# navallo/collision_avoidance

Measured on AMD Instinct MI355X. Metric: agent-steps/sec (whole node), 4096 arenas x 64 agents per GPU, higher is better.
Workload: dtype f32

## Files before the change

### collision_avoidance_amd/csrc/ca_obs.h

```cpp
#pragma once
#include "ca_common.h"

namespace ca {

struct ObsArgs {
    const float *pos_x, *pos_y, *vel_x, *vel_y, *orient_x, *orient_y;
    const unsigned short* counts;
    const void* nb_idx;
    const unsigned short* obst_idx;
    const ObstDev* obst;
    const int* tab_off;
    float* obs;
    int A, N, K, S, bpa;
    int nstage_max;
    int paircap;
    int a0;
    int xcd;
    int dense;
    unsigned long long* dbg;
    float radius;
    float rays[32];
    float oct[32];
    const float* ap_oct;
    const int* agent_counts;
};

#ifdef CA_STAMPS
#define CA_OSTAMP(k)                                                                       \
    do {                                                                                   \
        __builtin_amdgcn_sched_barrier(0);                                                 \
        const unsigned long long _t = CA_STAMP_CLOCK();                                    \
        __builtin_amdgcn_s_waitcnt(0xC07F);                                                \
        if ((threadIdx.x & 63) == 0 && p.dbg)                                              \
            p.dbg[((size_t)blockIdx.x * (blockDim.x >> 6) + (threadIdx.x >> 6)) * 16 + (k)] = _t; \
        __builtin_amdgcn_sched_barrier(0);                                                 \
    } while (0)
#else
#define CA_OSTAMP(k) do { } while (0)
#endif

__host__ __device__ inline size_t obs_lds_bytes(int nstage_max, int obs_bs, int paircap, int obw = 16) {
    const size_t apb = obs_bs / 16;
    return (size_t)nstage_max * 16 + 2 * apb * 16 * 8 + apb * 16 + apb * 16 * 4 + apb * (size_t)obw * 4 + 64 * 4 + 2 * apb * 4 + apb * (size_t)paircap * 2;
}
__host__ __device__ inline size_t obs_lds_bytes_ap(int nstage_max, int obs_bs, int paircap) {
    return ((obs_lds_bytes(nstage_max, obs_bs, paircap) + 15) & ~(size_t)15) + (size_t)(obs_bs / 16) * 16 * 64;
}
#ifndef CA_OBS_BS_MAX
#define CA_OBS_BS_MAX 256
#endif
__host__ __device__ inline int obs_block_threads(int N) {
    const int want = N > 32 ? 1024 : (N > 16 ? 512 : 256);
    return want < CA_OBS_BS_MAX ? want : CA_OBS_BS_MAX;
}

struct SegGeom {
    float s02x, s02y;
    float s32x, s32y;
    float t_numer;
    float r1x, r1y, r2x, r2y;
};

__device__ __forceinline__ float ray_dial(float x, float y) {
    const float yy = -y;
    const float ax = fabsf(x), ay = fabsf(yy);
    const float mx = fmaxf(ax, ay), mn = fminf(ax, ay);
    const float a = mn * __builtin_amdgcn_rcpf(mx);
    const float s = a * a;
    float r = a * (0.99997726f + s * (-0.33262347f + s * (0.19354346f + s * (-0.11643287f +
              s * (0.05265332f + s * -0.01172120f)))));
    r = (ay > ax) ? 1.57079632679f - r : r;
    r = (x < 0.0f) ? 3.14159265359f - r : r;
    r = (yy < 0.0f) ? -r : r;
    const float u = r * 2.54647908947f;
    return (u < 0.0f) ? u + 16.0f : u;
}

template <int OBS_BS, bool NW16, bool DENSE = false, class... WIDE_TAG>
__global__ __launch_bounds__(OBS_BS) void obs_kernel(const ObsArgs p) {
    constexpr bool WIDE = has_tag<WideObstLists, WIDE_TAG...>;
    constexpr bool AC = has_tag<ArenaCounts, WIDE_TAG...>;
    constexpr bool AP = has_tag<AgentParams, WIDE_TAG...> || AC;
    static_assert(!(WIDE && AP), "per-agent parameters go with obstacle lists of up to 16");
    constexpr int OBS_APB = OBS_BS / 16;
    extern __shared__ float4 smem4[];
    const int tid = threadIdx.x;
    const int g = tid >> 4, r = tid & 15;
    const int N = p.N, K = p.K, S = p.S;
    const int PAIRCAP = p.paircap;
    int bid = blockIdx.x;
    if (p.xcd) { const int x = bid & 7, idx = bid >> 3, q8 = idx / p.bpa; bid = (x + 8 * q8) * p.bpa + (idx - q8 * p.bpa); }
    int a, i, a_lo, nstage;
    bool active;
    if constexpr (DENSE) {
        const int first = bid * OBS_APB, gi = first + g;
        active = gi < p.A * N;
        const int ga = active ? gi : p.A * N - 1;
        a = p.a0 + ga / N; i = ga - (ga / N) * N;
        a_lo = p.a0 + first / N;
        const int last = min(first + OBS_APB - 1, p.A * N - 1);
        nstage = (last / N - first / N + 1) * N;
    } else {
        const int ab = bid / p.bpa;
        a = p.a0 + ab;
        i = (bid - ab * p.bpa) * OBS_APB + g;
        active = i < N;
        a_lo = a; nstage = N;
    }
    const int abase = DENSE ? (a - a_lo) * N : 0;
    const size_t q = (size_t)a * N + (active ? i : 0);
    const size_t aoff = (size_t)a * N;
    const unsigned ii = active ? (unsigned)i : 0u;
    const ObstDev* tab = p.obst + (p.tab_off ? p.tab_off[a] : 0);

    const int NST = p.nstage_max;
    float* s_px = reinterpret_cast<float*>(smem4);
    float* s_py = s_px + NST;
    float* s_vx = s_py + NST;
    float* s_vy = s_vx + NST;
    unsigned long long* s_key = reinterpret_cast<unsigned long long*>(s_vy + NST);
    float2* s_rel = reinterpret_cast<float2*>(s_key + OBS_APB * 16);
    float4* s_frame = reinterpret_cast<float4*>(s_rel + OBS_APB * 16);
    int* s_nb = reinterpret_cast<int*>(s_frame + OBS_APB);
    int* s_ob = s_nb + OBS_APB * 16;
    const int OBW = WIDE ? S : 16;
    float* s_rays = reinterpret_cast<float*>(s_ob + OBS_APB * OBW);
    float* s_oct = s_rays + 32;
    int* s_cnt = reinterpret_cast<int*>(s_oct + 32);
    int* s_cnt2 = s_cnt + OBS_APB;
    unsigned short* s_pair = reinterpret_cast<unsigned short*>(s_cnt2 + OBS_APB);
    const int SPAIRS = 16 * S;
    float2* s_noct = reinterpret_cast<float2*>(reinterpret_cast<char*>(smem4) + ((obs_lds_bytes(NST, OBS_BS, PAIRCAP) + 15) & ~(size_t)15));
    CA_OSTAMP(0);
    if (tid < 32) { s_rays[tid] = p.rays[tid]; s_oct[tid] = p.oct[tid]; }

    constexpr bool GATHER = NW16;
    const float* gpx = p.pos_x + (size_t)a * N;
    const float* gpy = p.pos_y + (size_t)a * N;
    const float* gvx = p.vel_x + (size_t)a * N;
    const float* gvy = p.vel_y + (size_t)a * N;
    if constexpr (!GATHER) {
        if constexpr (DENSE) {
            for (int t = tid; t < nstage; t += OBS_BS) {
                const size_t qa = (size_t)a_lo * N + t;
                s_px[t] = p.pos_x[qa]; s_py[t] = p.pos_y[qa]; s_vx[t] = p.vel_x[qa]; s_vy[t] = p.vel_y[qa];
            }
        } else {
            for (unsigned t = tid; t < (unsigned)nstage; t += OBS_BS) {
                s_px[t] = (p.pos_x + aoff)[t]; s_py[t] = (p.pos_y + aoff)[t]; s_vx[t] = (p.vel_x + aoff)[t]; s_vy[t] = (p.vel_y + aoff)[t];
            }
        }
    }
    int nn = 0, ns = 0;
    float c = 1.0f, s = 0.0f;
    if (active) {
        if constexpr (DENSE) {
            const int cnts = p.counts[q];
            nn = cnts & 0xFF; ns = cnts >> 8;
            if constexpr (AC) { if (i >= p.agent_counts[a]) { nn = 0; ns = 0; } }
            c = p.orient_x[q]; s = -p.orient_y[q];
            if (r < nn) s_nb[g * 16 + r] = abase + ld_idx_t<NW16>(p.nb_idx, ((size_t)a * K + r) * N + i);
            if constexpr (WIDE) { for (int t = r; t < ns; t += 16) s_ob[g * OBW + t] = (int)p.obst_idx[((size_t)a * S + t) * N + i]; }
            else if (r < ns) s_ob[g * 16 + r] = (int)p.obst_idx[((size_t)a * S + r) * N + i];
        } else {
            const int cnts = (p.counts + aoff)[ii];
            nn = cnts & 0xFF; ns = cnts >> 8;
            if constexpr (AC) { if (i >= p.agent_counts[a]) { nn = 0; ns = 0; } }
            c = (p.orient_x + aoff)[ii]; s = -(p.orient_y + aoff)[ii];
            const unsigned li = (unsigned)r * (unsigned)N + ii;
            const char* nbase = (const char*)p.nb_idx + aoff * (size_t)K * (NW16 ? 2 : 1);
            if (r < nn) s_nb[g * 16 + r] = ld_idx_t<NW16>(nbase, li);
            if constexpr (WIDE) { for (unsigned t = (unsigned)r; t < (unsigned)ns; t += 16u) s_ob[g * OBW + t] = (int)(p.obst_idx + aoff * (size_t)S)[t * (unsigned)N + ii]; }
            else if (r < ns) s_ob[g * 16 + r] = (int)(p.obst_idx + aoff * (size_t)S)[li];
        }
    }
    s_key[g * 16 + r] = ~0ull;
    if (r == 0) { s_cnt[g] = 0; s_cnt2[g] = 0; }
    CA_OSTAMP(1);
    __syncthreads();
    CA_OSTAMP(2);

    const int M = 8 * nn + ns;
    float mx = 0.0f, my = 0.0f;
    if (M > 0) { mx = GATHER ? gpx[i] : s_px[abase + i]; my = GATHER ? gpy[i] : s_py[abase + i]; }
    if (r == 0) s_frame[g] = make_float4(c, s, mx, my);
    {
        const int k = r;
        int i0 = 0, w = 0;
        if (k < nn) {
            const int nb = s_nb[g * 16 + k];
            const float rx = (GATHER ? gpx[nb] : s_px[nb]) - mx, ry = (GATHER ? gpy[nb] : s_py[nb]) - my;
            s_rel[g * 16 + k] = make_float2(rx, ry);
            float Rk = p.radius;
            if constexpr (AP) {
                const size_t nq = (DENSE ? (size_t)a_lo * N : aoff) + (size_t)nb;
                const float2* src = reinterpret_cast<const float2*>(p.ap_oct) + nq * 8;
                float2* dst = s_noct + (g * 16 + k) * 8;
#pragma unroll
                for (int e = 0; e < 8; ++e) dst[e] = src[e];
                Rk = src[0].x;
            }
            const float d2 = rx * rx + ry * ry, R = Rk;
            const float ax = c * rx - s * ry, ay = s * rx + c * ry;
            const bool all = !(d2 > 1.0404f * R * R);
            const float ua = ray_dial(ax, ay);
            const float t = R * __builtin_amdgcn_rsqf(d2);
            const float t2 = t * t;
            const float hw = t * (1.0f + t2 * (0.16666667f + t2 * (0.075f + t2 * 0.32914f))) * 2.54647908947f + 0.002f;
            int i1 = (int)floorf(ua + hw);
            i0 = (int)ceilf(ua - hw);
            if (all || i1 - i0 >= 15) { i0 = 0; i1 = 15; }
            w = max(i1 - i0 + 1, 0);
        }
        const int incl = wave_prefix_sum(w);
        int base = 0;
        if ((tid & 63) == 63) base = atomicAdd(&s_cnt[0], incl);
        base = __builtin_amdgcn_readlane(base, 63) + (incl - w);
        const unsigned short hd = (unsigned short)((g << 8) | (k << 4));
#pragma unroll
        for (int t2 = 0; t2 < 4; ++t2)
            if (t2 < w) s_pair[base + t2] = (unsigned short)(hd | ((i0 + t2) & 15));
        if (__builtin_expect(__ballot(w > 4) != 0ull, 0)) {
#pragma clang loop vectorize(disable) unroll(disable)
            for (int t2 = 4; t2 < w; ++t2) s_pair[base + t2] = (unsigned short)(hd | ((i0 + t2) & 15));
        }
    }
    {
        const float dx = s_rays[2 * r], dy = s_rays[2 * r + 1];
        int cnt2 = 0;
        for (int sidx = 0; sidx < ns; ++sidx) {
            const ObstDev o1 = load_obst(tab, s_ob[g * OBW + sidx]);
            const float x1 = o1.px - mx, y1 = o1.py - my, x2 = o1.qx - mx, y2 = o1.qy - my;
            const float ax = c * x1 - s * y1, ay = s * x1 + c * y1;
            const float bx = c * x2 - s * y2, by = s * x2 + c * y2;
            const float c2 = dx * ay - dy * ax, c3 = dx * by - dy * bx;
            const float f2 = dx * ax + dy * ay, f3 = dx * bx + dy * by;
            const float tolE = 1e-5f * p.rays[0] * (fabsf(ax) + fabsf(ay) + fabsf(bx) + fabsf(by) + 1.0f);
            const bool keep = !(c2 > tolE && c3 > tolE) && !(c2 < -tolE && c3 < -tolE) && (fmaxf(f2, f3) >= -tolE);
            const unsigned grp = (unsigned)(__ballot(keep) >> (threadIdx.x & 48)) & 0xFFFFu;
            if (keep)
                s_pair[OBS_APB * PAIRCAP - 1 - (g * SPAIRS + cnt2 + __popc(grp & ((1u << r) - 1u)))] =
                    (unsigned short)(((nn + sidx) << 4) | r);
            cnt2 += __popc(grp);
        }
        if (r == 0) s_cnt2[g] = cnt2;
    }
    CA_OSTAMP(3);
    __syncthreads();
    CA_OSTAMP(4);
    auto build = [&](int m, SegGeom& sg, float& velx, float& vely, bool want_vel) {
        float x1, y1, x2, y2, vx = 0.0f, vy = 0.0f;
        if (m < 8 * nn) {
            const int k = m >> 3, e = m & 7;
            const float2 rel = s_rel[g * 16 + k];
            const float rx = rel.x, ry = rel.y;
            if constexpr (AP) {
                const float2 va = s_noct[(g * 16 + k) * 8 + e], vb = s_noct[(g * 16 + k) * 8 + ((e + 1) & 7)];
                x1 = va.x + rx; y1 = va.y + ry;
                x2 = vb.x + rx; y2 = vb.y + ry;
            } else {
                const float4 oc = reinterpret_cast<const float4*>(s_oct)[e];
                x1 = oc.x + rx; y1 = oc.y + ry;
                x2 = oc.z + rx; y2 = oc.w + ry;
            }
            if (want_vel) { const int nb = s_nb[g * 16 + k]; vx = GATHER ? gvx[nb] : s_vx[nb]; vy = GATHER ? gvy[nb] : s_vy[nb]; }
        } else {
            const ObstDev o1 = load_obst(tab, s_ob[g * OBW + (m - 8 * nn)]);
            x1 = o1.px - mx; y1 = o1.py - my;
            x2 = o1.qx - mx; y2 = o1.qy - my;
        }
        sg.r1x = c * x1 - s * y1; sg.r1y = s * x1 + c * y1;
        sg.r2x = c * x2 - s * y2; sg.r2y = s * x2 + c * y2;
        sg.s32x = sg.r2x - sg.r1x; sg.s32y = sg.r2y - sg.r1y;
        sg.s02x = 0.0f - sg.r1x; sg.s02y = 0.0f - sg.r1y;
        sg.t_numer = sg.s32x * sg.s02y - sg.s32y * sg.s02x;
        if (want_vel) {
            const float lvx = x1 + vx, lvy = y1 + vy;
            const float rvx = c * lvx - s * lvy, rvy = s * lvx + c * lvy;
            velx = rvx - sg.r1x; vely = rvy - sg.r1y;
        }
    };
    auto build_nb = [&](const float2& fr, float rx, float ry, int e, SegGeom& sg, int slot) {
        float x1, y1, x2, y2;
        if constexpr (AP) {
            const float2 va = s_noct[slot * 8 + e], vb = s_noct[slot * 8 + ((e + 1) & 7)];
            x1 = va.x + rx; y1 = va.y + ry; x2 = vb.x + rx; y2 = vb.y + ry;
        } else {
            const float4 oc = reinterpret_cast<const float4*>(s_oct)[e];
            x1 = oc.x + rx; y1 = oc.y + ry; x2 = oc.z + rx; y2 = oc.w + ry;
        }
        sg.r1x = fr.x * x1 - fr.y * y1; sg.r1y = fr.y * x1 + fr.x * y1;
        sg.r2x = fr.x * x2 - fr.y * y2; sg.r2y = fr.y * x2 + fr.x * y2;
        sg.s32x = sg.r2x - sg.r1x; sg.s32y = sg.r2y - sg.r1y;
        sg.s02x = 0.0f - sg.r1x; sg.s02y = 0.0f - sg.r1y;
        sg.t_numer = sg.s32x * sg.s02y - sg.s32y * sg.s02x;
    };
    auto hit = [&](const SegGeom& sg, float s10x, float s10y, float& d, float& hx, float& hy) -> bool {
        const float denom = s10x * sg.s32y - sg.s32x * s10y;
        if (denom == 0.0f) return false;
        const bool dpos = denom > 0.0f;
        const float s_numer = s10x * sg.s02y - s10y * sg.s02x;
        if ((s_numer < 0.0f) == dpos) return false;
        if ((sg.t_numer < 0.0f) == dpos) return false;
        if (((s_numer > denom) == dpos) || ((sg.t_numer > denom) == dpos)) return false;
        const float t = div_ir(sg.t_numer, denom);
        hx = 0.0f + t * s10x; hy = 0.0f + t * s10y;
        d = sqrt_ir(hx * hx + hy * hy);
        return true;
    };

    auto accept_nb = [&](const SegGeom& sg, float s10x, float s10y, float& denom) -> bool {
        denom = s10x * sg.s32y - sg.s32x * s10y;
        const float s_numer = s10x * sg.s02y - s10y * sg.s02x;
        const bool dpos = denom > 0.0f;
        return (denom != 0.0f) && ((s_numer < 0.0f) != dpos) && ((sg.t_numer < 0.0f) != dpos) &&
               ((s_numer > denom) != dpos) && ((sg.t_numer > denom) != dpos);
    };
    auto hit_dist = [&](float t_numer, float denom, float s10x, float s10y) -> float {
        const float t = div_ir(t_numer, denom);
        const float hx = 0.0f + t * s10x, hy = 0.0f + t * s10y;
        return sqrt_ir(hx * hx + hy * hy);
    };

    const float tol_u = 2e-5f * p.rays[0] * (p.rays[0] + 2.0f * p.radius + 1.0f);
    auto merge = [&](int ga, int ray, float best, int best_m) {
        if (best_m >= 0)
            atomicMin(&s_key[ga * 16 + ray], ((unsigned long long)__float_as_uint(best) << 32) | (unsigned)best_m);
    };
    const int ntot = s_cnt[0];
    for (int pi = tid; pi < ntot; pi += OBS_BS) {
        const int pr = s_pair[pi];
        const int ga = pr >> 8, k = (pr >> 4) & 15, ray = pr & 15;
        const float2 fr = *reinterpret_cast<const float2*>(&s_frame[ga]);
        const float2 rel = s_rel[pr >> 4];
        const float s10x = s_rays[2 * ray] - 0.0f, s10y = s_rays[2 * ray + 1] - 0.0f;
        float best = __int_as_float(0x7f800000);
        int best_m = -1;
        const float rx = rel.x, ry = rel.y;
        const float wx = fr.x * s10x + fr.y * s10y, wy = fr.x * s10y - fr.y * s10x;
        const float wb = wx * ry - wy * rx;
        float Rp = p.radius, tol = tol_u;
        if constexpr (AP) {
            Rp = s_noct[(pr >> 4) * 8].x;
            tol = 2e-5f * p.rays[0] * (p.rays[0] + 2.0f * Rp + 1.0f);
        }
        const float R = Rp, Rh = 0.70710678f * R;
        const float c0 = R * wy, c2 = R * wx, c1 = Rh * (wx + wy), c3 = Rh * (wy - wx);
        const float cr[8] = {wb - c0, wb - c1, wb - c2, wb + c3, wb + c0, wb + c1, wb + c2, wb - c3};
        unsigned acc = 0;
#pragma unroll
        for (int e = 0; e < 8; ++e) {
            const float ca = cr[e], cb = cr[(e + 1) & 7];
            const bool same_side = (ca > tol && cb > tol) || (ca < -tol && cb < -tol);
            acc |= same_side ? 0u : (1u << e);
        }
        while (acc) {
            const int e1 = __ffs(acc) - 1;
            acc &= acc - 1;
            const bool two = acc != 0;
            const int e2 = two ? __ffs(acc) - 1 : e1;
            acc &= acc - 1;
            SegGeom g1, g2;
            build_nb(fr, rx, ry, e1, g1, pr >> 4);
            build_nb(fr, rx, ry, e2, g2, pr >> 4);
            float dn1, dn2;
            const bool ok1 = accept_nb(g1, s10x, s10y, dn1), ok2 = accept_nb(g2, s10x, s10y, dn2) && two;
            const float lhs = fabsf(g1.t_numer) * fabsf(dn2), rhs = fabsf(g2.t_numer) * fabsf(dn1);
            const bool first = ok1 && (!ok2 || lhs < rhs);
            const float tnw = first ? g1.t_numer : g2.t_numer, dnw = first ? dn1 : dn2;
            const int ew = first ? e1 : e2;
            const bool sure = fminf(lhs, rhs) < 0.99999f * fmaxf(lhs, rhs) && fmaxf(lhs, rhs) > 1e-30f &&
                              fabsf(tnw) > 1e-12f * fabsf(dnw);
            if (ok1 && ok2 && !sure) {
                const float d1 = hit_dist(g1.t_numer, dn1, s10x, s10y), d2 = hit_dist(g2.t_numer, dn2, s10x, s10y);
                if (d1 < best) { best = d1; best_m = 8 * k + e1; }
                if (d2 < best) { best = d2; best_m = 8 * k + e2; }
            } else {
                const float dw = hit_dist(tnw, dnw, s10x, s10y);
                if ((ok1 || ok2) && dw < best) { best = dw; best_m = 8 * k + ew; }
            }
        }
        merge(ga, ray, best, best_m);
    }
    const int no = s_cnt2[g];
    for (int pi = r; pi < no; pi += 16) {
        const int pr = s_pair[OBS_APB * PAIRCAP - 1 - (g * SPAIRS + pi)];
        const int k = pr >> 4, ray = pr & 15;
        const float s10x = s_rays[2 * ray] - 0.0f, s10y = s_rays[2 * ray + 1] - 0.0f;
        SegGeom sg;
        float dum0, dum1, d, hx, hy;
        const int m = 8 * nn + (k - nn);
        build(m, sg, dum0, dum1, false);
        if (hit(sg, s10x, s10y, d, hx, hy)) merge(g, ray, d, m);
    }
    CA_OSTAMP(5);
    __syncthreads();
    CA_OSTAMP(6);
    if (!active) return;
    const unsigned long long key = s_key[g * 16 + r];
    float bx = 0.0f, by = 0.0f, vx = 0.0f, vy = 0.0f;
    if (key != ~0ull) {
        SegGeom sg;
        float wx, wy;
        build((int)(unsigned)key, sg, wx, wy, true);
        const float s10x = s_rays[2 * r] - 0.0f, s10y = s_rays[2 * r + 1] - 0.0f;
        const float t = div_ir(sg.t_numer, s10x * sg.s32y - sg.s32x * s10y);
        bx = 0.0f + t * s10x; by = 0.0f + t * s10y;
        if (!(bx == 0.0f && by == 0.0f)) { vx = wx; vy = wy; }
    }
    CA_OSTAMP(7);
    {
        typedef float v4f __attribute__((ext_vector_type(4)));
        const v4f out = {bx, by, vx, vy};
        if constexpr (DENSE) __builtin_nontemporal_store(out, reinterpret_cast<v4f*>(p.obs) + (q * 16 + r));
        else __builtin_nontemporal_store(out, (reinterpret_cast<v4f*>(p.obs) + aoff * 16) + (ii * 16u + (unsigned)r));
    }
    CA_OSTAMP(8);
}

}
```

Before: 2.417 billion.

## Deal neighbor windows and wall items across all block threads instead of per agent

Neighbor-window candidate generation is redistributed so each thread handles one (agent, neighbor) slot using a reciprocal-multiply divide by K, which compacts work into fewer wavefronts instead of leaving lanes idle when nn<16. Wall/obstacle segments are compacted into an LDS work list through wave ballots and atomics, then processed block-wide with one lane per (segment, ray) pair. This replaces the per-agent serial wall loop and the pair list. The obstacle table offset is folded into the stored indices. The change adds LDS atomics, extra LDS state and indirection through the frame array, and relies on s_item fitting within the pair buffer.

After: 2.476 billion (median of 6 runs). +2.4%, better.

```diff
diff --git a/collision_avoidance_amd/csrc/ca_obs.h b/collision_avoidance_amd/csrc/ca_obs.h
--- a/collision_avoidance_amd/csrc/ca_obs.h
+++ b/collision_avoidance_amd/csrc/ca_obs.h
@@ -39,9 +39,17 @@
 #define CA_OSTAMP(k) do { } while (0)
 #endif
 
+#ifndef CA_OBS_DEAL_WINDOWS
+#define CA_OBS_DEAL_WINDOWS 1
+#endif
+#ifndef CA_OBS_DEAL_WALLS
+#define CA_OBS_DEAL_WALLS 1
+#endif
+
 __host__ __device__ inline size_t obs_lds_bytes(int nstage_max, int obs_bs, int paircap, int obw = 16) {
     const size_t apb = obs_bs / 16;
-    return (size_t)nstage_max * 16 + 2 * apb * 16 * 8 + apb * 16 + apb * 16 * 4 + apb * (size_t)obw * 4 + 64 * 4 + 2 * apb * 4 + apb * (size_t)paircap * 2;
+    return (size_t)nstage_max * 16 + 2 * apb * 16 * 8 + apb * 16 + apb * 16 * 4 + apb * (size_t)obw * 4 + 64 * 4 + 2 * apb * 4 + apb * (size_t)paircap * 2 +
+           ((CA_OBS_DEAL_WINDOWS && !CA_OBS_DEAL_WALLS) ? apb * 4 : 0);
 }
 __host__ __device__ inline size_t obs_lds_bytes_ap(int nstage_max, int obs_bs, int paircap) {
     return ((obs_lds_bytes(nstage_max, obs_bs, paircap) + 15) & ~(size_t)15) + (size_t)(obs_bs / 16) * 16 * 64;
@@ -90,7 +98,9 @@
     const int PAIRCAP = p.paircap;
     int bid = blockIdx.x;
     if (p.xcd) { const int x = bid & 7, idx = bid >> 3, q8 = idx / p.bpa; bid = (x + 8 * q8) * p.bpa + (idx - q8 * p.bpa); }
+    constexpr bool DEAL_WINDOWS = CA_OBS_DEAL_WINDOWS != 0, DEAL_WALLS = CA_OBS_DEAL_WALLS != 0;
     int a, i, a_lo, nstage;
+    int sbase;
     bool active;
     if constexpr (DENSE) {
         const int first = bid * OBS_APB, gi = first + g;
@@ -98,12 +108,14 @@
         const int ga = active ? gi : p.A * N - 1;
         a = p.a0 + ga / N; i = ga - (ga / N) * N;
         a_lo = p.a0 + first / N;
+        sbase = first - (first / N) * N;
         const int last = min(first + OBS_APB - 1, p.A * N - 1);
         nstage = (last / N - first / N + 1) * N;
     } else {
         const int ab = bid / p.bpa;
         a = p.a0 + ab;
-        i = (bid - ab * p.bpa) * OBS_APB + g;
+        sbase = (bid - ab * p.bpa) * OBS_APB;
+        i = sbase + g;
         active = i < N;
         a_lo = a; nstage = N;
     }
@@ -111,7 +123,7 @@
     const size_t q = (size_t)a * N + (active ? i : 0);
     const size_t aoff = (size_t)a * N;
     const unsigned ii = active ? (unsigned)i : 0u;
-    const ObstDev* tab = p.obst + (p.tab_off ? p.tab_off[a] : 0);
+    const int toff = p.tab_off ? p.tab_off[a] : 0;
 
     const int NST = p.nstage_max;
     float* s_px = reinterpret_cast<float*>(smem4);
@@ -130,6 +142,8 @@
     int* s_cnt2 = s_cnt + OBS_APB;
     unsigned short* s_pair = reinterpret_cast<unsigned short*>(s_cnt2 + OBS_APB);
     const int SPAIRS = 16 * S;
+    unsigned short* s_item = s_pair + OBS_APB * PAIRCAP - OBS_APB * S;
+    int* s_nn = DEAL_WALLS ? s_cnt2 : reinterpret_cast<int*>(s_pair + OBS_APB * PAIRCAP);
     float2* s_noct = reinterpret_cast<float2*>(reinterpret_cast<char*>(smem4) + ((obs_lds_bytes(NST, OBS_BS, PAIRCAP) + 15) & ~(size_t)15));
     CA_OSTAMP(0);
     if (tid < 32) { s_rays[tid] = p.rays[tid]; s_oct[tid] = p.oct[tid]; }
@@ -160,8 +174,8 @@
             if constexpr (AC) { if (i >= p.agent_counts[a]) { nn = 0; ns = 0; } }
             c = p.orient_x[q]; s = -p.orient_y[q];
             if (r < nn) s_nb[g * 16 + r] = abase + ld_idx_t<NW16>(p.nb_idx, ((size_t)a * K + r) * N + i);
-            if constexpr (WIDE) { for (int t = r; t < ns; t += 16) s_ob[g * OBW + t] = (int)p.obst_idx[((size_t)a * S + t) * N + i]; }
-            else if (r < ns) s_ob[g * 16 + r] = (int)p.obst_idx[((size_t)a * S + r) * N + i];
+            if constexpr (WIDE) { for (int t = r; t < ns; t += 16) s_ob[g * OBW + t] = toff + (int)p.obst_idx[((size_t)a * S + t) * N + i]; }
+            else if (r < ns) s_ob[g * 16 + r] = toff + (int)p.obst_idx[((size_t)a * S + r) * N + i];
         } else {
             const int cnts = (p.counts + aoff)[ii];
             nn = cnts & 0xFF; ns = cnts >> 8;
@@ -170,12 +184,17 @@
             const unsigned li = (unsigned)r * (unsigned)N + ii;
             const char* nbase = (const char*)p.nb_idx + aoff * (size_t)K * (NW16 ? 2 : 1);
             if (r < nn) s_nb[g * 16 + r] = ld_idx_t<NW16>(nbase, li);
-            if constexpr (WIDE) { for (unsigned t = (unsigned)r; t < (unsigned)ns; t += 16u) s_ob[g * OBW + t] = (int)(p.obst_idx + aoff * (size_t)S)[t * (unsigned)N + ii]; }
-            else if (r < ns) s_ob[g * 16 + r] = (int)(p.obst_idx + aoff * (size_t)S)[li];
+            if constexpr (WIDE) { for (unsigned t = (unsigned)r; t < (unsigned)ns; t += 16u) s_ob[g * OBW + t] = toff + (int)(p.obst_idx + aoff * (size_t)S)[t * (unsigned)N + ii]; }
+            else if (r < ns) s_ob[g * 16 + r] = toff + (int)(p.obst_idx + aoff * (size_t)S)[li];
         }
     }
     s_key[g * 16 + r] = ~0ull;
-    if (r == 0) { s_cnt[g] = 0; s_cnt2[g] = 0; }
+    if (r == 0) {
+        s_cnt[g] = 0;
+        if constexpr (!DEAL_WALLS) s_cnt2[g] = 0;
+        s_frame[g] = make_float4(c, s, 0.0f, 0.0f);
+        if constexpr (DEAL_WINDOWS || DEAL_WALLS) s_nn[g] = nn;
+    }
     CA_OSTAMP(1);
     __syncthreads();
     CA_OSTAMP(2);
@@ -183,11 +202,38 @@
     const int M = 8 * nn + ns;
     float mx = 0.0f, my = 0.0f;
     if (M > 0) { mx = GATHER ? gpx[i] : s_px[abase + i]; my = GATHER ? gpy[i] : s_py[abase + i]; }
-    if (r == 0) s_frame[g] = make_float4(c, s, mx, my);
-    {
-        const int k = r;
+    if (r == 0) reinterpret_cast<float2*>(&s_frame[g])[1] = make_float2(mx, my);
+    if constexpr (DEAL_WALLS) {
+        for (int t = r; ; t += 16) {
+            const bool has = t < ns;
+            const unsigned long long bal = __ballot(has);
+            if (bal == 0ull) break;
+            int base = 0;
+            if ((tid & 63) == 0) base = atomicAdd(&s_cnt[1], __popcll(bal));
+            base = __builtin_amdgcn_readfirstlane(base);
+            const int rank = (int)__builtin_amdgcn_mbcnt_hi((unsigned)(bal >> 32), __builtin_amdgcn_mbcnt_lo((unsigned)bal, 0u));
+            if (has) s_item[base + rank] = (unsigned short)((g << 6) | t);
+            if constexpr (!WIDE) break;
+        }
+    }
+    static constexpr unsigned RCP_K[17] = {0, 65537, 32769, 21846, 16385, 13108, 10923, 9363, 8193, 7282, 6554, 5958, 5462, 5042, 4682, 4370, 4097};
+    if (!DEAL_WINDOWS || __builtin_amdgcn_readfirstlane(tid & ~63) < OBS_APB * K) {
+        int gw = g, k = r;
+        bool live = r < nn;
+        float wc = c, ws = s, wmx = mx, wmy = my;
+        if constexpr (DEAL_WINDOWS) {
+            gw = (int)(((unsigned)tid * RCP_K[K]) >> 16); k = tid - gw * K;
+            live = tid < OBS_APB * K && k < s_nn[tid < OBS_APB * K ? gw : 0];
+            if (live) {
+                const float2 cs = *reinterpret_cast<const float2*>(&s_frame[gw]);
+                wc = cs.x; ws = cs.y;
+                wmx = GATHER ? gpx[sbase + gw] : s_px[sbase + gw]; wmy = GATHER ? gpy[sbase + gw] : s_py[sbase + gw];
+            }
+        }
+        const float c = wc, s = ws, mx = wmx, my = wmy;
+        const int g = gw;
         int i0 = 0, w = 0;
-        if (k < nn) {
+        if (live) {
             const int nb = s_nb[g * 16 + k];
             const float rx = (GATHER ? gpx[nb] : s_px[nb]) - mx, ry = (GATHER ? gpy[nb] : s_py[nb]) - my;
             s_rel[g * 16 + k] = make_float2(rx, ry);
@@ -225,11 +271,11 @@
             for (int t2 = 4; t2 < w; ++t2) s_pair[base + t2] = (unsigned short)(hd | ((i0 + t2) & 15));
         }
     }
-    {
+    if constexpr (!DEAL_WALLS) {
         const float dx = s_rays[2 * r], dy = s_rays[2 * r + 1];
         int cnt2 = 0;
         for (int sidx = 0; sidx < ns; ++sidx) {
-            const ObstDev o1 = load_obst(tab, s_ob[g * OBW + sidx]);
+            const ObstDev o1 = load_obst(p.obst, s_ob[g * OBW + sidx]);
             const float x1 = o1.px - mx, y1 = o1.py - my, x2 = o1.qx - mx, y2 = o1.qy - my;
             const float ax = c * x1 - s * y1, ay = s * x1 + c * y1;
             const float bx = c * x2 - s * y2, by = s * x2 + c * y2;
@@ -265,7 +311,7 @@
             }
             if (want_vel) { const int nb = s_nb[g * 16 + k]; vx = GATHER ? gvx[nb] : s_vx[nb]; vy = GATHER ? gvy[nb] : s_vy[nb]; }
         } else {
-            const ObstDev o1 = load_obst(tab, s_ob[g * OBW + (m - 8 * nn)]);
+            const ObstDev o1 = load_obst(p.obst, s_ob[g * OBW + (m - 8 * nn)]);
             x1 = o1.px - mx; y1 = o1.py - my;
             x2 = o1.qx - mx; y2 = o1.qy - my;
         }
@@ -382,16 +428,37 @@
         }
         merge(ga, ray, best, best_m);
     }
-    const int no = s_cnt2[g];
-    for (int pi = r; pi < no; pi += 16) {
-        const int pr = s_pair[OBS_APB * PAIRCAP - 1 - (g * SPAIRS + pi)];
-        const int k = pr >> 4, ray = pr & 15;
-        const float s10x = s_rays[2 * ray] - 0.0f, s10y = s_rays[2 * ray + 1] - 0.0f;
-        SegGeom sg;
-        float dum0, dum1, d, hx, hy;
-        const int m = 8 * nn + (k - nn);
-        build(m, sg, dum0, dum1, false);
-        if (hit(sg, s10x, s10y, d, hx, hy)) merge(g, ray, d, m);
+    if constexpr (DEAL_WALLS) {
+        const int nlanes = 16 * s_cnt[1];
+        for (int t = tid; t < nlanes; t += OBS_BS) {
+            const int it = s_item[t >> 4];
+            const int ga = it >> 6, sl = it & 63;
+            const float4 fr = s_frame[ga];
+            const int m = 8 * s_nn[ga] + sl;
+            const ObstDev o1 = load_obst(p.obst, s_ob[ga * OBW + sl]);
+            const float x1 = o1.px - fr.z, y1 = o1.py - fr.w, x2 = o1.qx - fr.z, y2 = o1.qy - fr.w;
+            SegGeom sg;
+            sg.r1x = fr.x * x1 - fr.y * y1; sg.r1y = fr.y * x1 + fr.x * y1;
+            sg.r2x = fr.x * x2 - fr.y * y2; sg.r2y = fr.y * x2 + fr.x * y2;
+            sg.s32x = sg.r2x - sg.r1x; sg.s32y = sg.r2y - sg.r1y;
+            sg.s02x = 0.0f - sg.r1x; sg.s02y = 0.0f - sg.r1y;
+            sg.t_numer = sg.s32x * sg.s02y - sg.s32y * sg.s02x;
+            const float s10x = s_rays[2 * r] - 0.0f, s10y = s_rays[2 * r + 1] - 0.0f;
+            float d, hx, hy;
+            if (hit(sg, s10x, s10y, d, hx, hy)) merge(ga, r, d, m);
+        }
+    } else {
+        const int no = s_cnt2[g];
+        for (int pi = r; pi < no; pi += 16) {
+            const int pr = s_pair[OBS_APB * PAIRCAP - 1 - (g * SPAIRS + pi)];
+            const int k = pr >> 4, ray = pr & 15;
+            const float s10x = s_rays[2 * ray] - 0.0f, s10y = s_rays[2 * ray + 1] - 0.0f;
+            SegGeom sg;
+            float dum0, dum1, d, hx, hy;
+            const int m = 8 * nn + (k - nn);
+            build(m, sg, dum0, dum1, false);
+            if (hit(sg, s10x, s10y, d, hx, hy)) merge(g, ray, d, m);
+        }
     }
     CA_OSTAMP(5);
     __syncthreads();
```
